# epeters13/pyCuSDR

Measured on AMD Instinct MI355X. Metric: IQ Msamples/sec through Doppler matched-filter bank (256 bins, 2^20 chunk), higher is better.
Workload: dtype f32

## Files before the change

pycusdr_amd/csrc/mfbank.hip:

```cpp
#include <hip/hip_runtime.h>
#include <math.h>
#include <stdint.h>
#include <stdio.h>
#include <stdlib.h>
#include <string.h>
#include <atomic>
#include <condition_variable>
#include <deque>
#include <mutex>
#include <thread>
#include <vector>

#include "../../include/mfbank.h"
#include "fft_core.hpp"
#include "filter_taps.hpp"
#include "seg_kernels.hpp"
#include "wrap_kernels.hpp"
#include "twopass_kernels.hpp"
#include "small_kernels.hpp"
#include "sync_kernels.hpp"
#include "combine_kernels.hpp"
#include "energy_kernels.hpp"
#include "stream_kernels.hpp"
#include "clip_kernels.hpp"
#include "unpack_kernels.hpp"
#include "hostcopy.hpp"
#include "record_layout.hpp"

struct BlockFlight {
    bool active;
    int mode, nthreads, bcap, shift, op;
    int nb;
    RecordLayout lay;
    unsigned long long seq;
    bool clip;
};

constexpr int WG_NB = 32;
struct BlockGraph {
    hipGraph_t graph;
    hipGraphExec_t exec;
    mfb_block_params params;
    int nb;
    unsigned long long epoch;
    bool seen, failed;
};

struct mfb_ctx {
    int device;
    int log2N, N, N1, N2, l1, l2, lo;
    int D, Doff, Dtot, M, W, sum_all, cs_off;
    int chunk, mpb, jsplit;
    int MU;
    bool chunk_auto;
    int *d_uniq, *d_rep;
    int parts, srb;
    int num_cus;
    hipStream_t own_stream, stream;
    cf *h_in;
    uint8_t *h_back;
    size_t back_cap;
    cf *h_X;
    bool mirror, mirror_valid;
    hipStream_t copy_stream;
    hipEvent_t ev_fft, ev_X;
    cf *d_x, *d_X, *d_masks, *d_Z, *d_xc, *d_P;
    const cf *d_in;
    float *d_env;
    int *d_shifts;
    cf *d_tw1, *d_tw2, *d_twLo, *d_twHi;
    float *d_part, *d_sum, *d_res, *d_cr;
    int *d_sym, *d_cen;
    float *d_mag;
    int cap;
    size_t z_rows;
    bool have_filters, have_shifts, have_input, have_xc;
    hipEvent_t t0, t1;
    bool prof;
    int path_req, segl_req;
    int path, segl;
    int T, win_start, V, Q;
    int seg_wpc, seg_mpb;
    cf *d_G, *d_twL;
    int twL_len;
    size_t part_cap;
    taps::Bank *bank;
    int basis_req, basis;
    int MB;
    cf *d_Gb;
    int gb_l;
    int search_mode;
    float *d_pow, *d_W;
    cf *h_in2;
    cf *d_x2;
    hipStream_t in_stream;
    hipEvent_t ev_h2d[2];
    hipEvent_t ev_xfree[2];
    uint8_t *h_blk[2];
    size_t blk_cap[2];
    hipEvent_t ev_blk[2];
    BlockFlight flight[2];
    unsigned long long blk_seq;
    BlockGraph bgraph[2][2];
    unsigned long long epoch;
    uint8_t *d_blkout;
    uint8_t *d_blkout2;
    BlockGraph bgraph2[2][2];
    BlockScalars *d_scal;
    int band_cap;
    bool W_valid;
    int win_blocks, win_stride;
    cf *h_win[2], *d_win[2];
    hipEvent_t ev_wh2d[2], ev_wfree[2];
    int bat_cap;
    cf *d_Xb, *d_xcb, *d_Pb;
    float *d_envb, *d_sumb, *d_resb, *d_crb;
    uint8_t *d_batout;
    uint8_t *d_batout2;
    size_t batout_cap;
    hipStream_t s2;
    hipEvent_t ev_p1[2];
    cf *d_Z2;
    size_t z2_rows;
    bool use_z2;
    bool s2_busy;
    bool batch_overlap;
    int last_batch_blocks;
    int cu_part, cu_parts;
    BlockGraph wgraph2[2][2][2][WG_NB + 1];
    BlockGraph wgraph[2][2][2][WG_NB + 1];
    bool st_on;
    StreamArgs st;
    uint8_t *d_lut8;
    int *d_lut3;
    int8_t *d_sttmpl;
    StreamCarry *d_carry[2];
    int carry_cur;
    StreamCarry *h_seed;
    std::vector<hipEvent_t> ev[2];
    std::vector<hipEvent_t> ev_pool;
    std::vector<int> h_shifts, h_uniq;
    std::vector<int> h_mult;
    float *d_Qs = nullptr;
    cf *d_Gs = nullptr;
// ... 225 lines not shown
    const int b = (int)SegCfg<L>::lds_bytes(L == 8192 ? 8 : SEG_MPB_MAX);
    HIPCHK(hipFuncSetAttribute((const void *)k_seg<L, SEG_STORE, -1>, hipFuncAttributeMaxDynamicSharedMemorySize, b));
#define MFB_ATTR_PV(PV_) HIPCHK(hipFuncSetAttribute((const void *)k_seg<L, SEG_REDUCE, PV_>, hipFuncAttributeMaxDynamicSharedMemorySize, b))
    MFB_ATTR_PV(-1);
    if constexpr (seg_ppl(L) == 32) {
        MFB_ATTR_PV(16); MFB_ATTR_PV(17); MFB_ATTR_PV(18); MFB_ATTR_PV(19); MFB_ATTR_PV(20); MFB_ATTR_PV(21); MFB_ATTR_PV(22);
        MFB_ATTR_PV(23); MFB_ATTR_PV(24); MFB_ATTR_PV(25); MFB_ATTR_PV(26); MFB_ATTR_PV(27); MFB_ATTR_PV(28); MFB_ATTR_PV(29);
        MFB_ATTR_PV(30); MFB_ATTR_PV(31); MFB_ATTR_PV(32);
    } else {
        MFB_ATTR_PV(8);
        MFB_ATTR_PV(9);
        MFB_ATTR_PV(10);
        MFB_ATTR_PV(11);
        MFB_ATTR_PV(12);
        MFB_ATTR_PV(13);
        MFB_ATTR_PV(14);
        MFB_ATTR_PV(15);
        MFB_ATTR_PV(16);
    }
#undef MFB_ATTR_PV
    return MFB_OK;
}
static int set_kernel_attributes(const mfb_ctx *c) {
    int rc = MFB_OK;
    switch (c->l1) {
        case 5: rc = attr_p1<32>(); break;
        case 6: rc = attr_p1<64>(); break;
        case 7: rc = attr_p1<128>(); break;
        case 8: rc = attr_p1<256>(); break;
        case 9: rc = attr_p1<512>(); break;
    }
    if (rc) return rc;
    switch (c->l2) {
        case 13: rc = attr_p2<8192>(); break;
        default: break;
    }
    if (rc) return rc;
    if ((rc = attr_seg<256>())) return rc;
    {
        const int b = (int)(SegCfg<256>::LDS_ELEMS * sizeof(cf) + (size_t)(SegCfg<256>::BLOCK / 64) * SEG_MPB_MAX * SEG_ACC_STRIDE * sizeof(float));
#define MFB_ATTR_F(PV_) HIPCHK(hipFuncSetAttribute((const void *)k_segf<256, PV_>, hipFuncAttributeMaxDynamicSharedMemorySize, b))
        MFB_ATTR_F(8); MFB_ATTR_F(9); MFB_ATTR_F(10); MFB_ATTR_F(11); MFB_ATTR_F(12); MFB_ATTR_F(13); MFB_ATTR_F(14); MFB_ATTR_F(15); MFB_ATTR_F(16);
#undef MFB_ATTR_F
#define MFB_ATTR_Q(L_, PV_, B_)                                                                                                       \
    if constexpr (segf_has_sumq<L_, PV_>())                                                                                           \
        HIPCHK(hipFuncSetAttribute((const void *)k_segf<L_, PV_, 1>, hipFuncAttributeMaxDynamicSharedMemorySize, B_));                    \
    if constexpr (segf_has_presum<L_, PV_>())                                                                                         \
        HIPCHK(hipFuncSetAttribute((const void *)k_segf<L_, PV_, 2>, hipFuncAttributeMaxDynamicSharedMemorySize, B_))
        MFB_ATTR_Q(256, 11, b); MFB_ATTR_Q(256, 12, b); MFB_ATTR_Q(256, 13, b); MFB_ATTR_Q(256, 14, b); MFB_ATTR_Q(256, 15, b);
        {
            const int bw = (int)SegWCfg<13, 3>::lds_bytes();
            HIPCHK(hipFuncSetAttribute((const void *)k_segw<13, 3>, hipFuncAttributeMaxDynamicSharedMemorySize, bw));
        }
        const int b2 = (int)(SegCfg<2048>::LDS_ELEMS * sizeof(cf) + (size_t)(SegCfg<2048>::BLOCK / 64) * 8 * SEG_ACC_STRIDE * sizeof(float));
#define MFB_ATTR_F(PV_) HIPCHK(hipFuncSetAttribute((const void *)k_segf<2048, PV_>, hipFuncAttributeMaxDynamicSharedMemorySize, b2))
        MFB_ATTR_F(16); MFB_ATTR_F(17); MFB_ATTR_F(18); MFB_ATTR_F(19); MFB_ATTR_F(20); MFB_ATTR_F(21); MFB_ATTR_F(22); MFB_ATTR_F(23); MFB_ATTR_F(24);
        MFB_ATTR_F(25); MFB_ATTR_F(26); MFB_ATTR_F(27); MFB_ATTR_F(28); MFB_ATTR_F(29); MFB_ATTR_F(30); MFB_ATTR_F(31); MFB_ATTR_F(32);
#undef MFB_ATTR_F
        MFB_ATTR_Q(2048, 22, b2); MFB_ATTR_Q(2048, 23, b2); MFB_ATTR_Q(2048, 24, b2); MFB_ATTR_Q(2048, 25, b2); MFB_ATTR_Q(2048, 26, b2);
        MFB_ATTR_Q(2048, 27, b2); MFB_ATTR_Q(2048, 28, b2); MFB_ATTR_Q(2048, 29, b2); MFB_ATTR_Q(2048, 30, b2); MFB_ATTR_Q(2048, 31, b2);
#undef MFB_ATTR_Q
    }
    if ((rc = attr_seg<512>())) return rc;
    if ((rc = attr_seg<1024>())) return rc;
    if ((rc = attr_seg<2048>())) return rc;
    if ((rc = attr_seg<4096>())) return rc;
    return attr_seg<8192>();
}

static int create_impl(mfb_ctx *c) {
    HIPCHK(hipStreamCreateWithFlags(&c->own_stream, hipStreamNonBlocking));
    c->stream = c->own_stream;
    HIPCHK(hipEventCreate(&c->t0));
    HIPCHK(hipEventCreate(&c->t1));
    int rc = set_kernel_attributes(c);
    if (rc) return rc;
    const int M = c->M;
    const size_t nb = (size_t)c->N * sizeof(cf);
    HIPCHK(hipHostMalloc((void **)&c->h_in, nb, hipHostMallocDefault));
    memset(c->h_in, 0, nb);
    c->back_cap = (size_t)3 * (c->N / 2) * sizeof(int) + ((size_t)256 << 10);
    if (c->back_cap < ((size_t)64 << 10)) c->back_cap = (size_t)64 << 10;
    HIPCHK(hipHostMalloc((void **)&c->h_back, c->back_cap, hipHostMallocDefault));
    HIPCHK(dev_alloc((void **)&c->d_x, nb));
    HIPCHK(dev_alloc((void **)&c->d_X, nb));
    HIPCHK(dev_alloc((void **)&c->d_masks, nb * M));
    HIPCHK(dev_alloc((void **)&c->d_xc, nb * M));
    HIPCHK(dev_alloc((void **)&c->d_P, nb));
    HIPCHK(dev_alloc((void **)&c->d_env, (size_t)c->N * sizeof(float)));
    HIPCHK(dev_alloc((void **)&c->d_shifts, (size_t)c->Dtot * sizeof(int)));
    if ((rc = reserve_partials(c, (size_t)c->Dtot * M * c->N1))) return rc;
    HIPCHK(dev_alloc((void **)&c->d_sum, (size_t)c->Dtot * M * sizeof(float)));
    HIPCHK(hipMemset(c->d_sum, 0, (size_t)c->Dtot * M * sizeof(float)));
    HIPCHK(dev_alloc((void **)&c->d_res, 2 * sizeof(float)));
    HIPCHK(dev_alloc((void **)&c->d_uniq, (size_t)M * sizeof(int)));
    HIPCHK(dev_alloc((void **)&c->d_rep, (size_t)M * sizeof(int)));
    HIPCHK(dev_alloc((void **)&c->d_cr, 3 * sizeof(float)));
    c->cap = c->N / 2;
    HIPCHK(dev_alloc((void **)&c->d_sym, (size_t)c->cap * sizeof(int)));
    HIPCHK(dev_alloc((void **)&c->d_cen, (size_t)c->cap * sizeof(int)));
    HIPCHK(dev_alloc((void **)&c->d_mag, (size_t)c->cap * sizeof(float)));
    if ((rc = alloc_Z(c))) return rc;
    if ((rc = blkout_reserve(c, 1024))) return rc;
    for (int i = 0; i < 2; ++i) {
        c->blk_cap[i] = rec_layout(c->band_cap, c->N / 3).bytes;
        HIPCHK(hipHostMalloc((void **)&c->h_blk[i], c->blk_cap[i], hipHostMallocDefault));
        HIPCHK(hipEventCreateWithFlags(&c->ev_blk[i], hipEventDisableTiming));
    }

    std::vector<cf> t;
    make_twiddles(t, c->N1, (double)c->N1, 1.0);
    if ((rc = upload_tw(&c->d_tw1, t))) return rc;
    make_twiddles(t, c->N2, (double)c->N2, 1.0);
    if ((rc = upload_tw(&c->d_tw2, t))) return rc;
    make_twiddles(t, 1 << c->lo, (double)c->N, 1.0);
    if ((rc = upload_tw(&c->d_twLo, t))) return rc;
    make_twiddles(t, c->N >> c->lo, (double)c->N, (double)(1 << c->lo));
    if ((rc = upload_tw(&c->d_twHi, t))) return rc;
    c->d_in = c->d_x;
    return MFB_OK;
}

static int create_body(mfb_ctx **out, int device, int log2N, int num_dopplers, int doppler_offset, int M,
                       int window_width, int sum_all_masks, int code_search_mask_offset) {
    if (!out) return MFB_ERR_ARG;
    *out = nullptr;
    if (num_dopplers < 1 || doppler_offset < 0 || M < 1 || M > 64 || window_width < 1 || (window_width & 1) == 0 ||
        code_search_mask_offset < 0 || 2 * code_search_mask_offset >= M)
        return MFB_ERR_ARG;
    if (log2N < 10 || log2N > 22) return MFB_ERR_UNSUPPORTED;
    int ndev = 0;
    HIPCHK(hipGetDeviceCount(&ndev));
    if (device < 0 || device >= ndev) return MFB_ERR_ARG;
    HIPCHK(hipSetDevice(device));
    int ncu = 0;
    HIPCHK(hipDeviceGetAttribute(&ncu, hipDeviceAttributeMultiprocessorCount, device));

    mfb_ctx *c = new mfb_ctx();
    memset((void *)c, 0, offsetof(mfb_ctx, ev));
    c->device = device;
    c->num_cus = ncu > 0 ? ncu : 256;
    c->log2N = log2N;
    c->N = 1 << log2N;
    c->l1 = log2N / 2 < 8 ? log2N / 2 : 8;
    if (log2N - c->l1 > 13) c->l1 = log2N - 13;
    c->l2 = log2N - c->l1;
    c->N1 = 1 << c->l1;
    c->N2 = 1 << c->l2;
    c->lo = (log2N + 1) / 2;
    c->D = num_dopplers;
    c->Doff = doppler_offset;
    c->Dtot = num_dopplers + doppler_offset;
    c->M = M;
    c->W = window_width;
    c->sum_all = sum_all_masks ? 1 : 0;
    c->cs_off = code_search_mask_offset;
    c->MU = M;
    c->chunk_auto = true;
    c->chunk = default_chunk(c);
    c->mpb = M < 8 ? M : 8;
    c->jsplit = 32;
    set_rows_per_block(c, 64);
    c->path_req = MFB_PATH_AUTO;
    c->path = MFB_PATH_TWOPASS;

    int rc;
    try {
        rc = create_impl(c);
    } catch (...) {
        (void)mfb_destroy(c);
        throw;
    }
    if (rc) {
        (void)mfb_destroy(c);
        return rc;
    }
    *out = c;
    return MFB_OK;
}
extern "C" int mfb_create(mfb_ctx **out, int device, int log2N, int num_dopplers, int doppler_offset, int M,
                          int window_width, int sum_all_masks, int code_search_mask_offset) {
    return guarded([&] { return create_body(out, device, log2N, num_dopplers, doppler_offset, M, window_width, sum_all_masks, code_search_mask_offset); });
}

static void graph_drop(BlockGraph &g);
template <class F>
static void for_each_graph(mfb_ctx *c, int slot, F &&f) {
    for (int in = 0; in < 2; ++in)
        for (int s = 0; s < 2; ++s) {
            if (slot >= 0 && s != slot) continue;
            f(c->bgraph[in][s]);
            f(c->bgraph2[in][s]);
            for (int par = 0; par < 2; ++par)
                for (int nb = 0; nb <= WG_NB; ++nb) {
                    f(c->wgraph[in][s][par][nb]);
                    f(c->wgraph2[in][s][par][nb]);
                }
        }
}
extern "C" int mfb_destroy(mfb_ctx *c) {
    if (!c) return MFB_ERR_ARG;
    (void)hipSetDevice(c->device);
    if (c->stream) (void)hipStreamSynchronize(c->stream);
    if (c->s2) (void)hipStreamSynchronize(c->s2);
    if (c->copy_stream) (void)hipStreamSynchronize(c->copy_stream);
    if (c->in_stream) (void)hipStreamSynchronize(c->in_stream);
    void *bufs[] = {c->d_uniq, c->d_rep, c->d_x,  c->d_X,    c->d_masks, c->d_Z,   c->d_xc,  c->d_P,   c->d_env, c->d_shifts, c->d_tw1,
                    c->d_tw2, c->d_twLo, c->d_twHi,  c->d_part, c->d_sum, c->d_res, c->d_cr,  c->d_sym,    c->d_cen, c->d_mag,
                    c->d_G, c->d_twL, c->d_Gb, c->d_pow, c->d_W, c->d_blkout, c->d_blkout2, c->d_x2,
                    c->d_win[0], c->d_win[1], c->d_Xb, c->d_xcb, c->d_Pb, c->d_envb, c->d_sumb, c->d_resb, c->d_crb, c->d_batout, c->d_batout2, c->d_Z2,
                    c->d_lut8, c->d_lut3, c->d_sttmpl, c->d_carry[0], c->d_carry[1]};
    for (void *p : bufs)
        if (p) (void)hipFree(p);
    if (c->h_in) (void)hipHostFree(c->h_in);
    if (c->h_in2) (void)hipHostFree(c->h_in2);
    for (int i = 0; i < 2; ++i) {
        if (c->h_win[i]) (void)hipHostFree(c->h_win[i]);
        if (c->ev_wh2d[i]) (void)hipEventDestroy(c->ev_wh2d[i]);
        if (c->ev_wfree[i]) (void)hipEventDestroy(c->ev_wfree[i]);
    }
    for_each_graph(c, -1, graph_drop);
    for (int i = 0; i < 2; ++i) {
        if (c->h_blk[i]) (void)hipHostFree(c->h_blk[i]);
        if (c->ev_blk[i]) (void)hipEventDestroy(c->ev_blk[i]);
        if (c->ev_p1[i]) (void)hipEventDestroy(c->ev_p1[i]);
    }
    if (c->s2) (void)hipStreamDestroy(c->s2);
    if (c->h_back) (void)hipHostFree(c->h_back);
    if (c->h_seed) (void)hipHostFree(c->h_seed);
    if (c->h_X) (void)hipHostFree(c->h_X);
    if (c->copy_stream) (void)hipStreamDestroy(c->copy_stream);
    if (c->in_stream) {
        (void)hipStreamSynchronize(c->in_stream);
        (void)hipStreamDestroy(c->in_stream);
    }
    for (int i = 0; i < 2; ++i) {
        if (c->ev_h2d[i]) (void)hipEventDestroy(c->ev_h2d[i]);
        if (c->ev_xfree[i]) (void)hipEventDestroy(c->ev_xfree[i]);
    }
    if (c->ev_fft) (void)hipEventDestroy(c->ev_fft);
    if (c->ev_X) (void)hipEventDestroy(c->ev_X);
    for (auto &v : c->ev)
        for (auto e : v) (void)hipEventDestroy(e);
    for (auto e : c->ev_pool) (void)hipEventDestroy(e);
    if (c->t0) (void)hipEventDestroy(c->t0);
    if (c->t1) (void)hipEventDestroy(c->t1);
    if (c->own_stream) (void)hipStreamDestroy(c->own_stream);
    if (c->d_Gs) (void)hipFree(c->d_Gs);
    if (c->d_Qs) (void)hipFree(c->d_Qs);
    if (c->d_Wb) (void)hipFree(c->d_Wb);
    if (c->d_Wexp) (void)hipFree(c->d_Wexp);
    for (int i = 0; i < 2; ++i) {
        if (c->d_clipx[i]) (void)hipFree(c->d_clipx[i]);
        if (c->d_clipi[i]) (void)hipFree(c->d_clipi[i]);
        if (c->d_cliph[i]) (void)hipFree(c->d_cliph[i]);
        if (c->h_cliph[i]) (void)hipHostFree(c->h_cliph[i]);
    }
    if (c->d_clips) (void)hipFree(c->d_clips);
    if (c->d_clipw) (void)hipFree(c->d_clipw);
    if (c->d_ctail) (void)hipFree(c->d_ctail);
    for (void *p : c->d_raw)
        if (p) (void)hipFree(p);
    delete c->bank;
    delete c;
    return MFB_OK;
}

extern "C" int mfb_set_stream(mfb_ctx *c, void *s) {
    if (!c) return MFB_ERR_ARG;
    HIPCHK(hipSetDevice(c->device));
    HIPCHK(sync_streams(c));
    c->stream = s ? (hipStream_t)s : c->own_stream;
    ++c->epoch;
    return MFB_OK;
}

extern "C" int mfb_set_cu_share(mfb_ctx *c, int part, int parts) {
    if (!c || parts < 1 || parts > 16 || part < 0 || part >= parts) return MFB_ERR_ARG;
    for (int s = 0; s < 2; ++s)
        if (c->flight[s].active) return MFB_ERR_STATE;
    HIPCHK(hipSetDevice(c->device));
    HIPCHK(sync_streams(c));
    hipStream_t fresh = nullptr;
    if (parts == 1) {
        HIPCHK(hipStreamCreateWithFlags(&fresh, hipStreamNonBlocking));
    } else {
        const int words = (c->num_cus + 31) / 32;
        std::vector<uint32_t> mask((size_t)words, 0u);
        int mine = 0;
        for (int i = 0; i < c->num_cus; ++i)
            if (i % parts == part) {
                mask[(size_t)i / 32] |= 1u << (i % 32);
                ++mine;
            }
        if (!mine) return MFB_ERR_ARG;
        HIPCHK(hipExtStreamCreateWithCUMask(&fresh, (uint32_t)words, mask.data()));
    }
    const bool was_own = c->stream == c->own_stream;
    if (c->own_stream) HIPCHK(hipStreamDestroy(c->own_stream));
    c->own_stream = fresh;
    if (was_own) c->stream = fresh;
    c->cu_part = part;
    c->cu_parts = parts;
    ++c->epoch;
    return MFB_OK;
}

extern "C" int mfb_set_tuning(mfb_ctx *c, int chunk, int mpb, int rows_per_block, int jsplit) {
    if (!c || chunk < 0 || mpb < 0 || rows_per_block < 0 || jsplit < 0) return MFB_ERR_ARG;
    ++c->epoch;
    HIPCHK(hipSetDevice(c->device));
// ... 676 lines not shown
    if (!c || !dev) return MFB_ERR_ARG;
    HIPCHK(hipSetDevice(c->device));
    c->d_in = (const cf *)dev;
    int rc = before_fft(c);
    if (rc) return rc;
    rc = forward_fft(c, c->d_in, nullptr, c->d_X);
    if (rc) return rc;
    if ((rc = after_fft(c))) return rc;
    c->have_input = true;
    c->have_xc = false;
    return MFB_OK;
}

static bool fsm_enabled() {
    static const int on = getenv("MFB_SEG_FSM") ? atoi(getenv("MFB_SEG_FSM")) : 1;
    return on != 0 && MFB_FFT_FUSED;
}
static bool wrap_mfma_enabled() {
    static const int on = getenv("MFB_SEG_WRAP_MFMA") ? atoi(getenv("MFB_SEG_WRAP_MFMA")) : 1;
    return on != 0;
}
static int wrap_kt(const mfb_ctx *c, bool span, int MU) {
    if (!wrap_mfma_enabled() || c->segl != 8 || c->N < (1 << 18) || !c->sum_all || !MFB_SEG_SUMQ || !c->bank || MU > 8) return 0;
    const bool presum = span || std::all_of(c->h_mult.begin(), c->h_mult.end(), [&](int m) { return m == c->h_mult[0]; });
    if (!presum || !segf_has_presum<256, 13>() || c->V != 13 * SegCfg<256>::NT) return 0;
    const int T = c->bank->T;
    return (T > 32 && T <= 48) ? 3 : 0;
}
static int fsm_prepare(mfb_ctx *c, bool span, int rows) {
    const int wkt = wrap_kt(c, span, rows);
    if (c->d_Gs && c->gs_rows == rows && c->gs_span == (span ? 1 : 0) && c->gs_l == c->segl && c->wb_kt == wkt) return MFB_OK;
    if ((int)c->h_shifts.size() != c->Dtot || !c->bank) return MFB_ERR_STATE;
    std::vector<float> G, Q;
    std::vector<uint16_t> W;
    std::vector<int> Wexp;
    std::vector<float> *q = (c->sum_all && MFB_SEG_SUMQ) ? &Q : nullptr;
    const int L = 1 << c->segl, Te = L - seg_valid(c->segl, c->bank->T) + 1;
    if (span) {
        taps::Bank sb;
        if (taps::span_basis(*c->bank, &sb) != rows) return MFB_ERR_STATE;
        taps::segment_spectra_shifted(sb, nullptr, rows, c->h_shifts.data(), c->Dtot, L, Te, &G, seg_ppl(L), q, nullptr);
        if (wkt) taps::wrap_taps_shifted(sb, nullptr, rows, c->h_shifts.data(), c->Dtot, wkt, &W, &Wexp);
    } else {
        if ((int)c->h_uniq.size() != rows || (int)c->h_mult.size() != rows || c->h_mult[0] < 1) return MFB_ERR_STATE;
        std::vector<double> wts((size_t)rows);
        for (int u = 0; u < rows; ++u) wts[(size_t)u] = (double)c->h_mult[(size_t)u] / (double)c->h_mult[0];
        taps::segment_spectra_shifted(*c->bank, c->h_uniq.data(), rows, c->h_shifts.data(), c->Dtot, L, Te, &G, seg_ppl(L), q, wts.data());
        if (wkt) taps::wrap_taps_shifted(*c->bank, c->h_uniq.data(), rows, c->h_shifts.data(), c->Dtot, wkt, &W, &Wexp);
    }
    HIPCHK(sync_streams(c));
    if (c->d_Gs) HIPCHK(hipFree(c->d_Gs));
    c->d_Gs = nullptr;
    c->gs_rows = 0;
    if (c->d_Qs) HIPCHK(hipFree(c->d_Qs));
    c->d_Qs = nullptr;
    if (c->d_Wb) HIPCHK(hipFree(c->d_Wb));
    c->d_Wb = nullptr;
    if (c->d_Wexp) HIPCHK(hipFree(c->d_Wexp));
    c->d_Wexp = nullptr;
    c->wb_kt = 0;
    HIPCHK(dev_alloc((void **)&c->d_Gs, G.size() * sizeof(float)));
    HIPCHK(hipMemcpy(c->d_Gs, G.data(), G.size() * sizeof(float), hipMemcpyHostToDevice));
    if (q) {
        HIPCHK(dev_alloc((void **)&c->d_Qs, Q.size() * sizeof(float)));
        HIPCHK(hipMemcpy(c->d_Qs, Q.data(), Q.size() * sizeof(float), hipMemcpyHostToDevice));
    }
    if (wkt) {
        HIPCHK(dev_alloc((void **)&c->d_Wb, W.size() * sizeof(uint16_t)));
        HIPCHK(hipMemcpy(c->d_Wb, W.data(), W.size() * sizeof(uint16_t), hipMemcpyHostToDevice));
        HIPCHK(dev_alloc((void **)&c->d_Wexp, Wexp.size() * sizeof(int)));
        HIPCHK(hipMemcpy(c->d_Wexp, Wexp.data(), Wexp.size() * sizeof(int), hipMemcpyHostToDevice));
        c->wb_kt = wkt;
    }
    c->gs_rows = rows;
    c->gs_span = span ? 1 : 0;
    c->gs_l = c->segl;
    return MFB_OK;
}
struct FsmPlan {
    bool ok, segw;
    int nsg, gbins, fb, fs, nbc, nsc;
};
constexpr int SEGW_FB = 32, SEGW_FS = 5;
static bool fsm_segw(const mfb_ctx *c, int MU) {
    return wrap_kt(c, c->basis == MFB_BASIS_SPAN, MU) == 3;
}
static FsmPlan fsm_plan(const mfb_ctx *c, int MU, int nfull, int nb = 1) {
    static int env_fb = 0, env_fs = 0;
    static const bool env_read = [] {
        const char *e = getenv("MFB_SEG_FSM_RECT");
        if (e) sscanf(e, "%d,%d", &env_fb, &env_fs);
        return true;
    }();
    (void)env_read;
    static const int env_gb = getenv("MFB_SEG_FSM_GROUP") ? atoi(getenv("MFB_SEG_FSM_GROUP")) : -1;
    FsmPlan p;
    memset(&p, 0, sizeof(p));
    const bool w32 = c->segl == 11;
    p.segw = fsm_segw(c, MU);
    p.nsg = nfull >= 64 ? 8 : 1;
    const int per_fwd = w32 ? 64 : 128;
    const bool fb_set = c->fsm_fb > 0 || env_fb > 0, fs_set = c->fsm_fs > 0 || env_fs > 0;
    int fb = c->fsm_fb > 0 ? c->fsm_fb : (env_fb > 0 ? env_fb : (per_fwd / MU > 2 ? per_fwd / MU : 2));
    int fs = c->fsm_fs > 0 ? c->fsm_fs : (env_fs > 0 ? env_fs : (p.segw ? SEGW_FS : 1));
    if (fb > c->Dtot) fb = c->Dtot;
    p.gbins = env_gb >= 0 ? (env_gb != 0) : (p.nsg > 1 && c->Dtot >= p.nsg * fb ? 1 : 0);
    if (p.gbins && c->Dtot < p.nsg) p.gbins = 0;
    if (w32 && !p.gbins && p.nsg > 1 && env_gb < 0) {
        fb = c->Dtot / p.nsg;
        if (fb < 1) return p;
        p.gbins = 1;
    }
    const int glen = p.gbins ? nfull : (nfull + p.nsg - 1) / p.nsg;
    const int gblen = p.gbins ? (c->Dtot + p.nsg - 1) / p.nsg : c->Dtot;
    if (p.segw && !fb_set) {
        const int chunks = (gblen + SEGW_FB - 1) / SEGW_FB;
        fb = (gblen + chunks - 1) / chunks;
    }
    if (fs > glen) fs = glen;
    if (fb > gblen) fb = gblen;
    if (fb < 1 || fs < 1) return p;
    auto waves = [&] { return (long long)nb * p.nsg * ((gblen + fb - 1) / fb) * ((glen + fs - 1) / fs); };
    if (p.segw) {
        const long long want = 4LL * c->num_cus;
        while (!fs_set && fs > 1 && waves() < want) fs = (fs + 1) >> 1;
        while (!fb_set && fb > 1 && waves() < want) fb = (fb + 1) >> 1;
    } else if (!fb_set) {
        const long long want = 2LL * c->num_cus * 4 * (w32 ? 2 : 3);
        while (fb > 1 && waves() < want) fb >>= 1;
    }
    p.fb = fb;
    p.fs = fs;
    p.nbc = (gblen + fb - 1) / fb;
    p.nsc = (glen + fs - 1) / fs;
    p.ok = true;
    return p;
}
template <int L, int PV0, int PV1>
static int launch_segf_pv(mfb_ctx *c, const SegFArgs &a, int grid, size_t lds, int pv) {
    if constexpr (PV0 > PV1) {
        return MFB_ERR_UNSUPPORTED;
    } else {
        if (pv == PV0) {
            bool done = false;
            if constexpr (segf_has_presum<L, PV0>()) {
                if (a.Qs && a.presum) {
                    hipLaunchKernelGGL((k_segf<L, PV0, 2>), dim3(grid), dim3(SegCfg<L>::BLOCK), lds, c->stream, a);
                    done = true;
                }
            }
            if constexpr (segf_has_sumq<L, PV0>()) {
                if (a.Qs && !done) {
                    hipLaunchKernelGGL((k_segf<L, PV0, 1>), dim3(grid), dim3(SegCfg<L>::BLOCK), lds, c->stream, a);
                    done = true;
                }
            }
            if (!done) hipLaunchKernelGGL((k_segf<L, PV0, 0>), dim3(grid), dim3(SegCfg<L>::BLOCK), lds, c->stream, a);
            HIPCHK(hipGetLastError());
            return MFB_OK;
        }
        return launch_segf_pv<L, PV0 + 1, PV1>(c, a, grid, lds, pv);
    }
}
static int launch_fsm(mfb_ctx *c, int nb, const cf *x, int xstride, int MU, int nfull, int parts, int pv) {
    SegFArgs a;
    memset(&a, 0, sizeof(a));
    a.x = x;
    a.Gs = c->d_Gs;
    a.Qs = c->sum_all ? c->d_Qs : nullptr;
    a.presum = c->gs_span == 1 || std::all_of(c->h_mult.begin(), c->h_mult.end(), [&](int m) { return m == c->h_mult[0]; }) ? 1 : 0;
    a.twL = c->d_twL;
    a.partials = c->d_part;
    a.N = c->N;
    a.V = c->V;
    a.slot0 = 0;
    a.nslots = nfull;
    a.MU = MU;
    a.dper = c->Dtot;
    a.nblk = nb;
    a.xstride = xstride;
    const FsmPlan fp = fsm_plan(c, MU, nfull, nb);
    if (!fp.ok) return MFB_ERR_UNSUPPORTED;
    a.nsg = fp.nsg;
    a.gbins = fp.gbins;
    a.fb = fp.fb;
    a.fs = fp.fs;
    a.nbc = fp.nbc;
// ... 146 lines not shown
        a.j0 = j0;
        a.dc = dc;
        a.M = MU;
        a.mpb = mpb;
        a.rows = (MU < c->M) ? c->d_uniq : nullptr;
        const int js = c->jsplit < dc ? c->jsplit : dc;
        a.ntiles = c->N2 / TILE;
        a.mgroups = mgroups;
        a.jsplit = js;
        prof_mark(c, 0);
        int rc = launch_p1<KIND_BANK>(c, a, dim3(a.ntiles * mgroups * js, 1, 1));
        prof_mark(c, 0);
        if (rc) return rc;
        P2Args b = p2_base(c);
        b.partials = c->d_part;
        b.part_row0 = j0 * MU;
        prof_mark(c, 1);
        rc = launch_p2<MODE_REDUCE>(c, b, dim3(c->parts, dc * MU, 1));
        prof_mark(c, 1);
        if (rc) return rc;
    }
    hipLaunchKernelGGL(k_finalize, dim3(c->Dtot), dim3(fin_threads(MU)), 0, c->stream, c->d_part, c->d_sum, c->Dtot, c->M, MU,
                       (const int *)c->d_rep, c->parts, c->sum_all);
    HIPCHK(hipGetLastError());
    return MFB_OK;
}

struct BackPiece {
    void *host;
    const void *dev;
    size_t bytes;
};
static int read_back(mfb_ctx *c, const BackPiece *p, int n) {
    size_t total = 0;
    for (int i = 0; i < n; ++i) total += (p[i].bytes + 15) & ~(size_t)15;
    const bool staged = c->h_back && total <= c->back_cap;
    size_t off = 0;
    for (int i = 0; i < n; ++i) {
        if (!p[i].bytes) continue;
        HIPCHK(hipMemcpyAsync(staged ? (void *)(c->h_back + off) : p[i].host, p[i].dev, p[i].bytes, hipMemcpyDeviceToHost, c->stream));
        off += (p[i].bytes + 15) & ~(size_t)15;
    }
    HIPCHK(sync_streams(c));
    if (staged) {
        off = 0;
        for (int i = 0; i < n; ++i) {
            if (p[i].bytes) memcpy(p[i].host, c->h_back + off, p[i].bytes);
            off += (p[i].bytes + 15) & ~(size_t)15;
        }
    }
    return MFB_OK;
}

extern "C" int mfb_export_scores_async(mfb_ctx *c, void *dst, int row_offset) {
    if (!c || !dst || row_offset < 0) return MFB_ERR_ARG;
    HIPCHK(hipSetDevice(c->device));
    HIPCHK(hipMemcpyAsync((float *)dst + (size_t)row_offset * c->M, c->d_sum, (size_t)c->Dtot * c->M * sizeof(float),
                          hipMemcpyDeviceToDevice, c->stream));
    return MFB_OK;
}

extern "C" int mfb_export_column_async(mfb_ctx *c, void *dst, int row_offset) {
    if (!c || !dst || row_offset < 0) return MFB_ERR_ARG;
    HIPCHK(hipSetDevice(c->device));
    HIPCHK(hipMemcpy2DAsync((float *)dst + row_offset, sizeof(float), c->d_sum, (size_t)c->M * sizeof(float), sizeof(float),
                            (size_t)c->Dtot, hipMemcpyDeviceToDevice, c->stream));
    return MFB_OK;
}

extern "C" int mfb_export_rows_async(mfb_ctx *c, void *dst, int dst_row, int first_row, int nrows, int column_only) {
    if (!c || !dst || dst_row < 0 || first_row < 0 || nrows < 0 || first_row + nrows > c->Dtot) return MFB_ERR_ARG;
    if (!nrows) return MFB_OK;
    HIPCHK(hipSetDevice(c->device));
    const float *src = c->d_sum + (size_t)first_row * c->M;
    if (column_only)
        HIPCHK(hipMemcpy2DAsync((float *)dst + dst_row, sizeof(float), src, (size_t)c->M * sizeof(float), sizeof(float), (size_t)nrows,
                                hipMemcpyDeviceToDevice, c->stream));
    else
        HIPCHK(hipMemcpyAsync((float *)dst + (size_t)dst_row * c->M, src, (size_t)nrows * c->M * sizeof(float), hipMemcpyDeviceToDevice,
                              c->stream));
    return MFB_OK;
}

extern "C" int mfb_pick_column(mfb_ctx *c, const void *column, int num, int offset, float res[2]) {
    if (!c || !column || !res || num < 1 || offset < 0) return MFB_ERR_ARG;
    if (!c->sum_all) return MFB_ERR_STATE;
    HIPCHK(hipSetDevice(c->device));
    hipLaunchKernelGGL(k_pick, dim3(1), dim3(64), 0, c->stream, (const float *)column, c->d_res, num, offset, 1, 1);
    HIPCHK(hipGetLastError());
    const BackPiece bp = {res, c->d_res, 2 * sizeof(float)};
    return read_back(c, &bp, 1);
}

extern "C" int mfb_pick(mfb_ctx *c, const void *scores, int num, int offset, float res[2]) {
    if (!c || !res || num < 1 || offset < 0) return MFB_ERR_ARG;
    if (!scores && (num != c->D || offset != c->Doff)) return MFB_ERR_ARG;
    HIPCHK(hipSetDevice(c->device));
    const float *in = scores ? (const float *)scores : c->d_sum;
    hipLaunchKernelGGL(k_pick, dim3(1), dim3(64), 0, c->stream, in, c->d_res, num, offset, c->M, c->sum_all);
    HIPCHK(hipGetLastError());
    const BackPiece bp = {res, c->d_res, 2 * sizeof(float)};
    return read_back(c, &bp, 1);
}

extern "C" int mfb_find_carrier(mfb_ctx *c, float res[2]) {
    int rc = mfb_search_async(c);
    if (rc) return rc;
    return mfb_pick(c, nullptr, c->D, c->Doff, res);
}

extern "C" int mfb_get_scores(mfb_ctx *c, float *host) {
    if (!c || !host) return MFB_ERR_ARG;
    HIPCHK(hipSetDevice(c->device));
    HIPCHK(hipMemcpyAsync(host, c->d_sum, (size_t)c->Dtot * c->M * sizeof(float), hipMemcpyDeviceToHost, c->stream));
    HIPCHK(sync_streams(c));
    return MFB_OK;
}

extern "C" int mfb_get_batch_scores(mfb_ctx *c, int block, float *host) {
    if (!c || !host || block < 0) return MFB_ERR_ARG;
    if (!c->d_sumb || block >= c->bat_cap || block >= c->last_batch_blocks) return MFB_ERR_STATE;
    HIPCHK(hipSetDevice(c->device));
    HIPCHK(sync_streams(c));
    HIPCHK(hipMemcpy(host, c->d_sumb + (size_t)block * c->Dtot * c->M, (size_t)c->Dtot * c->M * sizeof(float), hipMemcpyDeviceToHost));
    return MFB_OK;
}

extern "C" int mfb_get_spectrum(mfb_ctx *c, float *host, int start, int count) {
    if (!c || !host || count < 0 || count > c->N) return MFB_ERR_ARG;
    if (!c->have_input) return MFB_ERR_STATE;
    HIPCHK(hipSetDevice(c->device));
    start = ((start % c->N) + c->N) % c->N;
    const int first = (start + count <= c->N) ? count : c->N - start;
    if (c->mirror_valid) {
        HIPCHK(hipEventSynchronize(c->ev_X));
        memcpy(host, c->h_X + start, (size_t)first * sizeof(cf));
        if (first < count) memcpy(host + 2 * (size_t)first, c->h_X, (size_t)(count - first) * sizeof(cf));
        return MFB_OK;
    }
    const BackPiece bp[2] = {{host, c->d_X + start, (size_t)first * sizeof(cf)},
                             {host + 2 * (size_t)first, c->d_X, (size_t)(count - first) * sizeof(cf)}};
    const int rc = read_back(c, bp, 2);
    if (rc) return rc;
    return enable_mirror(c);
}

struct BlkBufs {
    int nb;
    const cf *x;
    int xstride;
    cf *X;
    float *sum;
    float *res;
    cf *xc;
    float *env;
    cf *P;
    float *cr;
    uint8_t *out;
    RecordLayout lay;
    bool batch;
    int parity;
    const struct ClipLaunch *clip;
};
static BlkBufs single_bufs(mfb_ctx *c, const RecordLayout &lay = RecordLayout{}) {
    return BlkBufs{1, c->d_in, 0, c->d_X, c->d_sum, c->d_res, c->d_xc, c->d_env, c->d_P, c->d_cr, c->d_blkout, lay, false, 0, nullptr};
}

static int demod_enqueue(mfb_ctx *c, const BlkBufs &bb, int shift, const int *shift_dev, int shift_stride, int k_offset, int k_len,
                         int spsym_min = 0, int capacity = 0, BlockScalars *scal = nullptr) {
    int rc;
    const int nb = bb.nb;
    if (c->path == MFB_PATH_SEGMENT) {
        int nfull, ntotal;
        seg_slots(c, &nfull, &ntotal);
        const bool fused_env = c->M <= SEG_MPB_MAX;
        const SegPlan p = plan_seg(c, nb, c->M, ntotal, fused_env ? c->M : 4);
        SegArgs sa = seg_base(c, p);
        sa.x = bb.x;
        sa.out = bb.xc;
        if (fused_env) {
            sa.env = bb.env;
            sa.env_lo = c->cs_off;
            sa.env_hi = c->M - c->cs_off;
        }
        sa.MU = c->M;
// ... 1996 lines not shown
```

pycusdr_amd/csrc/small_kernels.hpp:

```cpp
#pragma once
#include <stdint.h>

#include "fft_core.hpp"

#define FIN_MAX_ROWS 64
__global__ void __launch_bounds__(1024) k_finalize(const float *partials, float *dsum, int D, int M, int MU, const int *rep, int parts,
                                                   int sum_all) {
    __shared__ float srow[FIN_MAX_ROWS];
    const int j = blockIdx.x;
    const int lane = threadIdx.x & 63, wave = threadIdx.x >> 6, nw = blockDim.x >> 6;
    if (j >= D) return;
    for (int u = wave; u < MU; u += nw) {
        const float *p = partials + ((size_t)j * MU + u) * parts;
        float a0 = 0.f, a1 = 0.f, a2 = 0.f, a3 = 0.f;
        int q = lane;
        for (; q + 192 < parts; q += 256) {
            a0 += p[q];
            a1 += p[q + 64];
            a2 += p[q + 128];
            a3 += p[q + 192];
        }
        for (; q < parts; q += 64) a0 += p[q];
        float s = (a0 + a1) + (a2 + a3);
#pragma unroll
// ... 90 lines not shown
                        bidx = oi;
                    }
                }
                if (records > 0) {
                    const int gi = offset + gidx, bi = best > 0.f ? offset + bidx : 0;
                    if ((records - 1) & 1) {
                        mv1 = gmax, mi1 = gi, mv0 = best, mi0 = bi;
                    } else {
                        mv0 = gmax, mi0 = gi, mv1 = best, mi1 = bi;
                    }
                    cur = (mv0 >= mv1) ? 1 : 0;
                }
                closed = true;
            }
        }
        if (!closed) {
            mv0 = mv1 = 0.f;
            mi0 = mi1 = cur = 0;
            for (int r0 = offset; r0 < num + offset; r0 += 64) {
                const int r = r0 + lane;
                const bool inside = r < num + offset;
                const float v = inside ? in[(size_t)r * M + x] : 0.f;
                unsigned long long todo = ~0ull;
                while (true) {
                    const float thr = cur ? mv1 : mv0;
                    const unsigned long long hit = __ballot(inside && v > thr) & todo;
                    if (!hit) break;
                    const int l = __builtin_ctzll(hit);
                    const float tmp = __int_as_float(__builtin_amdgcn_readlane(__float_as_int(v), l));
                    if (cur) {
                        mv1 = tmp;
                        mi1 = r0 + l;
                    } else {
                        mv0 = tmp;
                        mi0 = r0 + l;
                    }
                    cur = (mv0 >= mv1) ? 1 : 0;
                    todo = (l == 63) ? 0ull : (~0ull << (l + 1));
                }
            }
        }
        const float numr = __fmaf_rn((float)mi0, mv0, __fmul_rn((float)mi1, mv1));
        const float idxL = __fdiv_rn(numr, __fadd_rn(mv0, mv1));
        float valL = __fdiv_rn(numr, (float)(mi0 + mi1));
        if (offset > 0) valL = __fdiv_rn(cur ? mv0 : mv1, in[x]);
        if (sum_all) {
            if (lane == 0) {
                res[0] = idxL;
                res[1] = 10.f * log10f(valL);
            }
            return;
        }
        if (lane == 0) {
            sIdx[x] = idxL;
            sVal[x] = valL;
        }
    }
    int n = 1;
    while (n < M) n <<= 1;
    __syncthreads();
    if (lane >= M) {
        sIdx[lane] = 0.f;
        sVal[lane] = 0.f;
    }
    __syncthreads();
    for (int step = n >> 1; step >= 1; step >>= 1) {
        float a = 0.f, b = 0.f;
        if (lane < n) {
            a = __fadd_rn(sIdx[lane], sIdx[lane ^ step]);
            b = __fadd_rn(sVal[lane], sVal[lane ^ step]);
        }
        __syncthreads();
        if (lane < n) {
            sIdx[lane] = a;
            sVal[lane] = b;
        }
        __syncthreads();
    }
    if (lane == 0) {
        res[0] = __fdiv_rn(sIdx[0], (float)M);
        res[1] = 10.f * log10f(__fdiv_rn(sVal[0], (float)M));
    }
}
__global__ void __launch_bounds__(64) k_pick(const float *in, float *res, int num, int offset, int M, int sum_all) {
    __shared__ float sIdx[64], sVal[64];
    __shared__ float scol[PICK_LDS];
    pick_body(in, res, num, offset, M, sum_all, sIdx, sVal, scol);
}

DEVI float abs2c(cf z) { return __fmaf_rn(z.x, z.x, __fmul_rn(z.y, z.y)); }

__global__ void k_envelope(const cf *xc, float *env, int N, int M, int off) {
    xc += (size_t)blockIdx.y * (size_t)M * (size_t)N;
    env += (size_t)blockIdx.y * (size_t)N;
    for (int x = blockIdx.x * blockDim.x + threadIdx.x; x < N; x += gridDim.x * blockDim.x) {
        float s = 0.f;
        for (int m = off; m < M - off; ++m) s = __fadd_rn(s, abs2c(xc[(size_t)m * N + x]));
        env[x] = s;
    }
}

DEVI void code_rate_body(const cf *P, float *out, int offset, int len, float *sv, int *si) {
    const int tid = threadIdx.x;
    unsigned emax = 0;
    for (int x = tid; x < len; x += blockDim.x) {
        const cf z = P[x + offset];
        const unsigned a = __float_as_uint(fabsf(z.x)), b = __float_as_uint(fabsf(z.y));
        if (a < 0x7f800000u && a > emax) emax = a;
        if (b < 0x7f800000u && b > emax) emax = b;
    }
    si[tid] = (int)emax;
    __syncthreads();
    for (int s = blockDim.x >> 1; s > 0; s >>= 1) {
        if (tid < s && (unsigned)si[tid + s] > (unsigned)si[tid]) si[tid] = si[tid + s];
        __syncthreads();
    }
    const int shift = 127 - (int)(((unsigned)si[0] >> 23) & 0xffu);
    __syncthreads();
    float best = -1.f;
    int bi = 0x7fffffff;
    for (int x = tid; x < len; x += blockDim.x) {
        const cf z = P[x + offset];
        const float v = abs2c(mkc(ldexpf(z.x, shift), ldexpf(z.y, shift)));
        if (v > best) {
            best = v;
            bi = x + offset;
        }
    }
    sv[tid] = best;
    si[tid] = bi;
    __syncthreads();
    for (int s = blockDim.x >> 1; s > 0; s >>= 1) {
        if (tid < s) {
            const float ov = sv[tid + s];
            const int oi = si[tid + s];
            if (ov > sv[tid] || (ov == sv[tid] && oi < si[tid])) {
                sv[tid] = ov;
                si[tid] = oi;
            }
        }
        __syncthreads();
    }
    if (tid == 0) {
        int k = (len > 0) ? si[0] : 0;
        if (len > 0 && (k < offset || k >= offset + len)) k = offset;
        const cf z = P[k];
        out[0] = (float)k;
        out[1] = atan2f(z.y, z.x);
        out[2] = (len > 0) ? abs2c(z) : -1.f;
    }
}
__global__ void k_code_rate(const cf *P, float *out, int offset, int len) {
    __shared__ float sv[1024];
    __shared__ int si[1024];
    code_rate_body(P, out, offset, len, sv, si);
}
DEVI void centres_body(int *outSym, int *outIdx, float *mag, const cf *sig, float spSym, float offset, int lenSig, int M, int W, int op,
                       int capacity, const int x) {
    if (x >= capacity) return;
    const float half = (float)(W / 2);
    const float base = __fmaf_rn((float)x, spSym, -half);
    int arrayIdx = (int)__fadd_rn(base, offset);
    int maxArrayIdx = arrayIdx + W;
    int offsetComp = (int)offset;
    if (arrayIdx < 0) {
        offsetComp -= arrayIdx;
        arrayIdx = 0;
    }
    if (maxArrayIdx > lenSig) maxArrayIdx = lenSig;
    maxArrayIdx -= arrayIdx;
// ... 205 lines not shown
```

Measured before the change: 2538.

## Add wide-group FSM segment plan and write pick result to pinned host memory

```diff
diff --git a/pycusdr_amd/csrc/mfbank.hip b/pycusdr_amd/csrc/mfbank.hip
--- a/pycusdr_amd/csrc/mfbank.hip
+++ b/pycusdr_amd/csrc/mfbank.hip
@@ -60,6 +60,7 @@
     cf *h_in;
     uint8_t *h_back;
     size_t back_cap;
+    float *h_pick, *h_pick_dev;
     cf *h_X;
     bool mirror, mirror_valid;
     hipStream_t copy_stream;
@@ -451,6 +452,8 @@
     c->back_cap = (size_t)3 * (c->N / 2) * sizeof(int) + ((size_t)256 << 10);
     if (c->back_cap < ((size_t)64 << 10)) c->back_cap = (size_t)64 << 10;
     HIPCHK(hipHostMalloc((void **)&c->h_back, c->back_cap, hipHostMallocDefault));
+    HIPCHK(hipHostMalloc((void **)&c->h_pick, 2 * sizeof(float), hipHostMallocDefault));
+    HIPCHK(hipHostGetDevicePointer((void **)&c->h_pick_dev, c->h_pick, 0));
     HIPCHK(dev_alloc((void **)&c->d_x, nb));
     HIPCHK(dev_alloc((void **)&c->d_X, nb));
     HIPCHK(dev_alloc((void **)&c->d_masks, nb * M));
@@ -596,6 +599,7 @@
     }
     if (c->s2) (void)hipStreamDestroy(c->s2);
     if (c->h_back) (void)hipHostFree(c->h_back);
+    if (c->h_pick) (void)hipHostFree(c->h_pick);
     if (c->h_seed) (void)hipHostFree(c->h_seed);
     if (c->h_X) (void)hipHostFree(c->h_X);
     if (c->copy_stream) (void)hipStreamDestroy(c->copy_stream);
@@ -1438,6 +1442,7 @@
     int nsg, gbins, fb, fs, nbc, nsc;
 };
 constexpr int SEGW_FB = 32, SEGW_FS = 5;
+constexpr int SEGW_WIDE_FB = 64, SEGW_WIDE_ROUNDS = 4;
 static bool fsm_segw(const mfb_ctx *c, int MU) {
     return wrap_kt(c, c->basis == MFB_BASIS_SPAN, MU) == 3;
 }
@@ -1459,6 +1464,25 @@
     const bool fb_set = c->fsm_fb > 0 || env_fb > 0, fs_set = c->fsm_fs > 0 || env_fs > 0;
     int fb = c->fsm_fb > 0 ? c->fsm_fb : (env_fb > 0 ? env_fb : (per_fwd / MU > 2 ? per_fwd / MU : 2));
     int fs = c->fsm_fs > 0 ? c->fsm_fs : (env_fs > 0 ? env_fs : (p.segw ? SEGW_FS : 1));
+    if (p.segw && !fb_set && env_gb < 0 && p.nsg > 1 && c->Dtot >= 4 * SEGW_FB) {
+        const int wnsg = c->Dtot <= 4 * SEGW_WIDE_FB ? 4 : 8;
+        const int share = (c->Dtot + wnsg - 1) / wnsg;
+        const int chunks = (share + SEGW_WIDE_FB - 1) / SEGW_WIDE_FB;
+        const long long want = (long long)SEGW_WIDE_ROUNDS * 4 * c->num_cus;
+        auto wwaves = [&](int s) { return (long long)nb * wnsg * chunks * ((nfull + s - 1) / s); };
+        if (wwaves(1) >= want) {
+            if (fs > nfull) fs = nfull;
+            while (!fs_set && fs > 1 && wwaves(fs) < want) --fs;
+            p.nsg = wnsg;
+            p.gbins = 1;
+            p.fb = (share + chunks - 1) / chunks;
+            p.fs = fs;
+            p.nbc = (share + p.fb - 1) / p.fb;
+            p.nsc = (nfull + fs - 1) / fs;
+            p.ok = true;
+            return p;
+        }
+    }
     if (fb > c->Dtot) fb = c->Dtot;
     p.gbins = env_gb >= 0 ? (env_gb != 0) : (p.nsg > 1 && c->Dtot >= p.nsg * fb ? 1 : 0);
     if (p.gbins && c->Dtot < p.nsg) p.gbins = 0;
@@ -1771,14 +1795,20 @@
     return MFB_OK;
 }
 
+static int read_pick(mfb_ctx *c, float res[2]) {
+    HIPCHK(sync_streams(c));
+    res[0] = c->h_pick[0];
+    res[1] = c->h_pick[1];
+    return MFB_OK;
+}
+
 extern "C" int mfb_pick_column(mfb_ctx *c, const void *column, int num, int offset, float res[2]) {
     if (!c || !column || !res || num < 1 || offset < 0) return MFB_ERR_ARG;
     if (!c->sum_all) return MFB_ERR_STATE;
     HIPCHK(hipSetDevice(c->device));
-    hipLaunchKernelGGL(k_pick, dim3(1), dim3(64), 0, c->stream, (const float *)column, c->d_res, num, offset, 1, 1);
+    hipLaunchKernelGGL(k_pick, dim3(1), dim3(64), 0, c->stream, (const float *)column, c->d_res, c->h_pick_dev, num, offset, 1, 1);
     HIPCHK(hipGetLastError());
-    const BackPiece bp = {res, c->d_res, 2 * sizeof(float)};
-    return read_back(c, &bp, 1);
+    return read_pick(c, res);
 }
 
 extern "C" int mfb_pick(mfb_ctx *c, const void *scores, int num, int offset, float res[2]) {
@@ -1786,10 +1816,9 @@
     if (!scores && (num != c->D || offset != c->Doff)) return MFB_ERR_ARG;
     HIPCHK(hipSetDevice(c->device));
     const float *in = scores ? (const float *)scores : c->d_sum;
-    hipLaunchKernelGGL(k_pick, dim3(1), dim3(64), 0, c->stream, in, c->d_res, num, offset, c->M, c->sum_all);
+    hipLaunchKernelGGL(k_pick, dim3(1), dim3(64), 0, c->stream, in, c->d_res, c->h_pick_dev, num, offset, c->M, c->sum_all);
     HIPCHK(hipGetLastError());
-    const BackPiece bp = {res, c->d_res, 2 * sizeof(float)};
-    return read_back(c, &bp, 1);
+    return read_pick(c, res);
 }
 
 extern "C" int mfb_find_carrier(mfb_ctx *c, float res[2]) {
diff --git a/pycusdr_amd/csrc/small_kernels.hpp b/pycusdr_amd/csrc/small_kernels.hpp
--- a/pycusdr_amd/csrc/small_kernels.hpp
+++ b/pycusdr_amd/csrc/small_kernels.hpp
@@ -196,10 +196,14 @@
         res[1] = 10.f * log10f(__fdiv_rn(sVal[0], (float)M));
     }
 }
-__global__ void __launch_bounds__(64) k_pick(const float *in, float *res, int num, int offset, int M, int sum_all) {
+__global__ void __launch_bounds__(64) k_pick(const float *in, float *res, float *hres, int num, int offset, int M, int sum_all) {
     __shared__ float sIdx[64], sVal[64];
     __shared__ float scol[PICK_LDS];
     pick_body(in, res, num, offset, M, sum_all, sIdx, sVal, scol);
+    if (threadIdx.x == 0) {
+        hres[0] = res[0];
+        hres[1] = res[1];
+    }
 }
 
 DEVI float abs2c(cf z) { return __fmaf_rn(z.x, z.x, __fmul_rn(z.y, z.y)); }
```

Result: faster. 2637 (median of 6 runs) (+3.9%).
